# Pyrokine/LineSegmentDetector-SLAM

Hardware: AMD Instinct MI355X
Metric: Mpixels/sec LSD (grad+grow+NFA) (higher is better)
Workload: dtype f64; 1 GPU; 512 x 2048x2048 u8 occupancy maps per GPU tiled/rolled/flipped from 4 aisle-class fixtures (SURVEY 8d C4), full pipeline incl. lineIm, params 0.3/0.6/22.5/0.7/1024; images_total=512, images_rank0=512, parallelism=single GPU, rccl_gather_in_step=False, steps_in_flight=8, steps_in_flight_asked=8, region_waves_per_image=4, help_across_workgroups=False, last_steps_with_help=0, writeback_map=False

## Files before the change

### linesegmentdetector-slam_amd/csrc/k_front.hip

```cpp
#include "lsd_internal.h"
#include "k_front_lds.h"
#include "k1_stage.h"
#include "grad_px.h"

namespace lsdhip {

constexpr int TW = kK1TileW, TH = kK1TileH, NT = 256;
constexpr int GW = kFrontGW, GH = kFrontGH;
constexpr int HS = 17, TAPR = 8;
constexpr int PPT = TW * TH / NT;
static_assert(TW == 32 && TW * TH % NT == 0, "a thread keeps its column and walks down the tile NT / TW rows at a time");

__global__ __launch_bounds__(NT, 4) void k_front(const uint8_t* __restrict__ in, double* __restrict__ mag, double* __restrict__ deg,
                                                 double2* __restrict__ sc, uint32_t* __restrict__ pw, unsigned long long* __restrict__ maxbits,
                                                 int32_t* __restrict__ ties, const double* __restrict__ taps_g, const int* __restrict__ centre_of,
                                                 int W, int H, int w, int h, double gradThre, int IWp, unsigned strip_bytes, unsigned gx,
                                                 unsigned gy, unsigned tiles, uint8_t* __restrict__ clr) {
    extern __shared__ __align__(16) unsigned char smem[];
    double* aux = reinterpret_cast<double*>(smem);
    double* taps = reinterpret_cast<double*>(smem + strip_bytes);
    uint8_t* tile = reinterpret_cast<uint8_t*>(taps + 3 * HS);
    double* Gt = reinterpret_cast<double*>(tile);
    int* l_cnt = reinterpret_cast<int*>(Gt + GW * GH);
    unsigned long long* l_max = reinterpret_cast<unsigned long long*>(l_cnt + 2);
    double2* l_g = reinterpret_cast<double2*>(smem);
    uint32_t* l_px = reinterpret_cast<uint32_t*>(l_g + kFrontList);

    const int tid = threadIdx.x;
    const unsigned per = (tiles + 7u) >> 3;
    const unsigned t = (blockIdx.x & 7u) * per + (blockIdx.x >> 3);
    if (t >= tiles) return;
    const unsigned bx = t % gx, tq = t / gx, by = tq % gy;
    const int X0 = (int)bx * TW, Y0 = (int)by * TH;
    const size_t img = tq / gy;
    const uint8_t* src = in + img * (size_t)W * H;
    const size_t base = img * (size_t)w * h;

    if (clr) {
        typedef uint32_t u32x4 __attribute__((ext_vector_type(4)));
        const unsigned tpi = gx * gy, ti = t % tpi;
        const size_t units = ((size_t)W * H) >> 4;
        const size_t a = units * ti / tpi, e = units * (ti + 1) / tpi;
        u32x4* const v = reinterpret_cast<u32x4*>(clr + img * (size_t)W * H);
        const u32x4 z = {0u, 0u, 0u, 0u};
        for (size_t u = a + tid; u < e; u += NT) __builtin_nontemporal_store(z, &v[u]);
    }
    const int Xf = max(X0 - 1, 0), Yf = max(Y0 - 1, 0);
    const int Xl = min(X0 + TW - 1, w - 1), Yl = min(Y0 + TH - 1, h - 1);
    const int c0 = centre_of[Xf] - TAPR, c1 = centre_of[Xl] + TAPR;
    const int r0 = centre_of[Yf] - TAPR, r1 = centre_of[Yl] + TAPR;
    const int IH = r1 - r0 + 1;

    for (int i = tid; i < 3 * HS; i += NT) taps[i] = taps_g[i];

    const int a0 = c0 - (((c0 % 4) + 4) % 4);
    const uint32_t wany = stage_window(src, tile, W, H, r0, r1, a0, c1, IWp, tid, 0u);

    const int X = tid & (TW - 1), Yt = tid / TW;
    const int gX = X0 + X;
    if (!__syncthreads_or((int)(wany != 0u))) {
        if (gX < w) {
            #pragma unroll
            for (int k = 0; k < PPT; k++) {
                const int gY = Y0 + Yt + k * (NT / TW);
                if (gY >= h) break;
                const GradPx px = grad_pixel(0.0, 0.0, 0.0, 0.0, gX >= 1 && gY >= 1, gradThre);
                const size_t p = base + (size_t)gY * w + gX;
                mag[p] = px.m;
                if (!px.heavy && px.u == 0) sc[p] = make_double2(0.0, 1.0);
                deg[p] = px.d;
                pw[p] = pack_pw(px.d, px.u);
            }
        }
        return;
    }
    const int DWp = IWp >> 2;
    if (gX < w) {
        const int cb = centre_of[gX] - TAPR - a0;
        const double* ker = taps + (gX % 3) * HS;
        double kr[HS];
        #pragma unroll
        for (int i = 0; i < HS; i++) kr[i] = ker[i];
        const uint32_t* trow = reinterpret_cast<const uint32_t*>(tile) + (cb >> 2);
        const uint32_t sh = (uint32_t)(cb & 3);
        for (int r = Yt; r < IH; r += NT / TW) aux[r * GW + 1 + X] = xpass17(trow + r * DWp, sh, kr);
    }
    if (X0 >= 1 && tid < IH) {
        const int cb = centre_of[X0 - 1] - TAPR - a0;
        const double* ker = taps + ((X0 - 1) % 3) * HS;
        double kr[HS];
        #pragma unroll
        for (int i = 0; i < HS; i++) kr[i] = ker[i];
        const uint32_t* trow = reinterpret_cast<const uint32_t*>(tile) + (cb >> 2);
        for (int r = tid; r < IH; r += NT) aux[r * GW] = xpass17(trow + r * DWp, (uint32_t)(cb & 3), kr);
    }
    __syncthreads();
    if (tid == 0) *l_cnt = 0;

    for (int idx = tid; idx < GW * GH; idx += NT) {
        const int Yh = idx / GW, Xh = idx - Yh * GW;
        const int gYh = Y0 - 1 + Yh, gXh = X0 - 1 + Xh;
        const bool ok = gYh >= 0 && gYh < h && gXh >= 0 && gXh < w;
        double v = 0;
        if (ok) {
            const int rb = centre_of[gYh] - TAPR - r0;
            const double* ker = taps + (gYh % 3) * HS;
            double a[HS];
            uint32_t bits = 0u;
            #pragma unroll
            for (int i = 0; i < HS; i++) { a[i] = aux[(rb + i) * GW + Xh]; bits |= (uint32_t)__double2hiint(a[i]) | (uint32_t)__double2loint(a[i]); }
            if (__ballot(bits != 0u) != 0ull) {
                #pragma unroll
                for (int i = 0; i < HS; i++) v += a[i] * ker[i];
            }
        }
        Gt[idx] = v;
    }
    __syncthreads();

    const int lane = tid & 63, wave = tid >> 6;
    const unsigned long long ltmask = (1ull << lane) - 1ull;
    double mx = 0;
    double rowD[PPT];
    uint32_t rowU[PPT];
    int rowSlot[PPT];
    #pragma unroll
    for (int k = 0; k < PPT; k++) {
        const int Y = Yt + k * (NT / TW), gY = Y0 + Y;
        const bool valid = gX < w && gY < h;
        const double* g1 = Gt + (Y + 1) * GW + X;
        const GradPx px = grad_pixel(g1[1], g1[0], g1[1 - GW], g1[-GW], valid && gX >= 1 && gY >= 1, gradThre);
        if (valid) {
            const size_t p = base + (size_t)gY * w + gX;
            mag[p] = px.m;
            if (!px.heavy && px.u == 0) sc[p] = make_double2(0.0, 1.0);
        }
        rowD[k] = px.d; rowU[k] = px.u; rowSlot[k] = -1;
        const unsigned long long hm = __ballot(px.heavy);
        if (hm != 0ull) {
            int b0 = 0;
            if (lane == 0) b0 = atomicAdd(l_cnt, __builtin_popcountll(hm));
            b0 = __builtin_amdgcn_readfirstlane(b0);
            if (px.heavy) {
                const int slot = b0 + __builtin_popcountll(hm & ltmask);
                l_px[slot] = ((uint32_t)(Y * TW + X) << 1) | (px.u == 0 ? 1u : 0u);
                l_g[slot] = make_double2(px.gradX, px.gradY);
                rowSlot[k] = slot;
            }
        }
        mx = fmax(mx, px.m);
    }
    {
        unsigned long long bits = (unsigned long long)__double_as_longlong(mx);
        for (int off = 32; off >= 1; off >>= 1) {
            const unsigned long long o = __shfl_xor(bits, off);
            bits = o > bits ? o : bits;
        }
        if (lane == 0) l_max[wave] = bits;
    }
    __syncthreads();
    if (tid == 0) {
        unsigned long long bits = l_max[0];
        #pragma unroll
        for (int i = 1; i < NT / 64; i++) bits = l_max[i] > bits ? l_max[i] : bits;
        if (bits != 0ull) atomicMax(&maxbits[img], bits);
    }

    const int cnt = *l_cnt;
    for (int i = tid; i < cnt; i += NT) {
        const uint32_t e = l_px[i];
        const double2 gr = l_g[i];
        const double d = grad_angle(gr.x, gr.y, &ties[img]);
        l_g[i] = make_double2(d, 0.0);
        if (e & 1u) {
            const int lt = (int)(e >> 1);
            sc[base + (size_t)(Y0 + lt / TW) * w + (X0 + lt % TW)] = grad_sincos(d);
        }
    }
    __syncthreads();

    if (gX < w) {
        #pragma unroll
        for (int k = 0; k < PPT; k++) {
            const int gY = Y0 + Yt + k * (NT / TW);
            if (gY < h) {
                const double d = rowSlot[k] >= 0 ? l_g[rowSlot[k]].x : rowD[k];
                const size_t p = base + (size_t)gY * w + gX;
                deg[p] = d;
                pw[p] = pack_pw(d, rowU[k]);
            }
        }
    }
}

bool front_fits(const Geom& g, size_t max_lds) {
    if (2 * g.tapR + 1 != HS) return false;
    const size_t need = k_front_lds(g.sca, g.tapR).bytes;
    return need <= 64 * 1024 && need <= max_lds;
}

void launch_front(const Geom& g, const Buffers& b, int n, uint8_t* clr, hipStream_t s) {
    const KFrontLds L = k_front_lds(g.sca, g.tapR);
    const unsigned gx = (g.w + TW - 1) / TW, gy = (g.h + TH - 1) / TH, tiles = gx * gy * (unsigned)n;
    hipLaunchKernelGGL(k_front, dim3(((tiles + 7u) >> 3) * 8u), dim3(NT), L.bytes, s, b.in, b.mag, b.deg, b.sc, b.pw, b.maxbits, b.ties, b.taps,
                       b.centres, g.W, g.H, g.w, g.h, g.gradThre, L.IWp, (unsigned)L.strip, gx, gy, tiles, clr);
}

}
```

### linesegmentdetector-slam_amd/csrc/k_front_lds.h

```cpp
#pragma once
#include <math.h>
#include <stddef.h>
#include "k1_lds.h"

namespace lsdhip {

constexpr int kFrontGW = kK1TileW + 1, kFrontGH = kK1TileH + 1;
constexpr int kFrontList = kK1TileW * kK1TileH;

struct KFrontLds {
    int IWp;
    int IHmax;
    size_t strip;
    size_t window;
    size_t bytes;
};

inline KFrontLds k_front_lds(double sca, int tapR) {
    KFrontLds r;
    const int span = (int)floor(kK1TileW / sca) + 2;
    const int IWmax = span + 2 * tapR + 1;
    r.IWp = ((IWmax + 3) & ~3) + 8;
    if (((r.IWp >> 2) & 1) == 0) r.IWp += 4;
    r.IHmax = (int)floor(kK1TileH / sca) + 2 + 2 * tapR + 1;
    const int hSize = 2 * tapR + 1;
    const size_t sums = (size_t)r.IHmax * kFrontGW * sizeof(double), list = (size_t)kFrontList * (16 + 4);
    const size_t win = ((size_t)r.IHmax * r.IWp + 7) & ~(size_t)7, post = (size_t)kFrontGW * kFrontGH * sizeof(double) + 8 + 4 * 8;
    r.strip = ((sums > list ? sums : list) + 15) & ~(size_t)15;
    r.window = win > post ? win : post;
    r.bytes = r.strip + 3 * (size_t)hSize * sizeof(double) + r.window;
    return r;
}

}
```

### linesegmentdetector-slam_amd/csrc/lsd_ctx.hip

```cpp
#include <math.h>
#include <stddef.h>
#include <stdio.h>
#include <stdlib.h>
#include <string.h>

#include <algorithm>
#include <mutex>
#include <string>
#include <vector>

#include "lsd_devbuf.h"
#include "lsd_internal.h"
#include "k1_lds.h"
#include "k_rdp_lds.h"

using namespace lsdhip;

struct Workspace {
    size_t cap_gpx = 0;
    size_t cap_n = 0, cap_npx = 0, cap_ws = 0;
    int cap_max_lines = 0;
    DevBuf<double> gauss, mag, deg, recs, recs_scaled;
    DevBuf<double2> sc;
    DevBuf<uint32_t> order;
    DevBuf<uint32_t> sets;
    DevBuf<uint32_t> pw, epochmap, ord, spill, gcopy, stamps, seedidx, seedpos, tepoch;
    uint32_t run_id = 0;
    DevBuf<uint32_t> slist;
    DevBuf<double> pend;
    DevBuf<float4> wmeta;
    DevBuf<int> rnum;
    DevBuf<uint32_t> xq;
    DevBuf<unsigned long long> maxbits;
    DevBuf<int32_t> nb, nseed;
    DevBuf<long long> stats;
    DevBuf<SeedRec> seeds;
    int32_t* ties() const { return reinterpret_cast<int32_t*>(maxbits.get() + cap_n); }
};

struct lsd_ctx {
    int device = 0;
    int num_cus = 256;
    size_t max_lds = 0;
    uint32_t id_budget = 0xFFFF0u;
    int tun_soft = 0, tun_claim = 0, tun_feed = 3, tun_big = 0;
    int tun_help = -1;
    int tun_gate = 12000;
    int tun_share = 0;
    int pool_max_images = 4;
    int tun_early = 0, tun_wb = 10, tun_up = 32, tun_down = 96, tun_requeue = 1, tun_xpoll = 20000, tun_linger = 1000000, tun_stop = 0;
    int region_waves_mode = 0;
    bool prefer4 = false;
    hipStream_t stream = nullptr;
    hipStream_t last_stream = nullptr;
    std::string err;
    Workspace ws;
    int mcap = 16384;
    int gcap = 8192;
    DevBuf<uint8_t> h_in, h_lineim;
    DevBuf<lsd_line> h_lines, h_flat;
    DevBuf<int32_t> h_counts, h_offs;
    uint8_t* pin[2] = {nullptr, nullptr};
    hipEvent_t pin_ev[2] = {nullptr, nullptr};
    bool pin_used[2] = {false, false};
    hipStream_t copy_stream = nullptr;
    size_t hcap_n = 0, hcap_wh = 0;
    int hcap_max_lines = 0;
    bool hcap_lineim = false;
    DevBuf<double> d_taps, d_lgamma, d_ptab;
    DevBuf<int> d_centres;
    bool cost_history = false;
    int hist_n = 0;
    lsd_params tab_params{};
    bool tab_valid = false;
    int tapR = 0;
    DevBuf<unsigned long long> mc_claim;
    DevBuf<uint32_t> mc_fa, mc_fb;
    DevBuf<int> mc_ctl;
    DevBuf<uint8_t> mc_in;
    DevBuf<double> mc_out;
    DevBuf<uint8_t> oc_in, oc_out;
    DevBuf<uint8_t> stage;
    DevBuf<uint8_t> fa_buf;
    DevBuf<uint8_t> gm_mr_ws;
    DevBuf<uint32_t> gr_volume;
    DevBuf<uint8_t> gm_slots;
    std::vector<int> fa_nf;
    std::vector<lsd_map_ref> map_tab_host = std::vector<lsd_map_ref>(2 * LSD_MAX_MAPS);
    DevBuf<lsd_map_ref> map_tab;
    int fa_lds_bound = kFaLdsMax;
    DevBuf<int32_t> ga_cnt;
    DevBuf<lsd_line> ga_slab;
    hipEvent_t ga_ev = nullptr;
    bool ga_ev_valid = false;
    int stop_after = 0;
    int tun_groups = -1;
    DevBuf<int> pcount;
    bool trace = false;
    bool fused_front = true;
    int scan_cap = kRdpShortMaxLen;
    bool rdp_long_ready = false;
    int host_max_lines = 8192;
    Geom geom{};
    int last_n = 0;
    int last_max_lines = 0;
    int32_t* last_counts = nullptr;
    bool last_fused = false, last_remapped = false;
    const uint8_t* last_in = nullptr;
    DevBuf<double> dbg_gauss;
    hipEvent_t ev[7]{};
    bool ev_valid = false;
    hipEvent_t ev_done = nullptr;
    bool done_valid = false;
    hipStream_t done_stream = nullptr;
};

constexpr size_t kPinBytes = 32u << 20;

#define HIPCHK(ctx, call)                                                                         \
    do {                                                                                          \
        hipError_t e_ = (call);                                                                   \
        if (e_ != hipSuccess) {                                                                   \
            (ctx)->err = std::string(#call) + ": " + hipGetErrorString(e_);                       \
            return e_ == hipErrorOutOfMemory ? LSD_ERR_NOMEM : LSD_ERR_HIP;                       \
        }                                                                                         \
    } while (0)

static int tap_radius(double sca, double sig) {
    const int prec = 3;
    if (sca < 1) sig = sig / sca;
    return cvt_x86(ceil(sig * sqrt(2 * prec * log(10))));
}

static void gauss_taps(double sca, double sig, int h, std::vector<double>& t) {
    if (sca < 1) sig = sig / sca;
    const int hSize = 1 + 2 * h;
    t.assign((size_t)3 * hSize, 0.0);
    double s1 = 0, s2 = 0, s3 = 0;
    for (int k = 0; k < hSize; k++) {
        const double a = (k - h) / sig, b = (k - h - 1.0 / 3) / sig, c = (k - h + 1.0 / 3) / sig;
        t[0 * hSize + k] = exp(-0.5 * (a * a));
        t[1 * hSize + k] = exp(-0.5 * (b * b));
        t[2 * hSize + k] = exp(-0.5 * (c * c));
        s1 += t[0 * hSize + k]; s2 += t[1 * hSize + k]; s3 += t[2 * hSize + k];
    }
    for (int k = 0; k < hSize; k++) {
        t[0 * hSize + k] /= s1; t[1 * hSize + k] /= s2; t[2 * hSize + k] /= s3;
    }
}

static double log_gamma_host(int x) {
    if (x > 15)
        return 0.918938533204673 + (x - 0.5) * log(x) - x + 0.5 * x * log(x * sinh(1.0 / x) + 1.0 / (810 * pow(x, 6)));
    static const double q[7] = {75122.6331530, 80916.6278952, 36308.2951477, 8687.24529705,
                                1168.92649479, 83.8676043424, 2.50662827511};
    double a = (x + 0.5) * log(x + 5.5) - (x + 5.5), b = 0;
    for (int i = 0; i < 7; i++) { a -= log(x + i); b += q[i] * pow(x, i); }
    return a + log(b);
}

static std::mutex g_lg_mu;
static const double* log_gamma_table(int count) {
    static std::vector<double> tab;
    if ((int)tab.size() < count) {
        const int from = (int)tab.size();
        tab.resize(count);
        for (int i = from; i < count; i++) tab[i] = i >= 1 ? log_gamma_host(i) : 0.0;
    }
    return tab.data();
}

static int make_geom(lsd_ctx* c, const lsd_params* p, int cols, int rows, Geom* g) {
    if (!p || cols <= 0 || rows <= 0) return LSD_ERR_INVALID;
    if (!(p->sca > 0) || !(p->sig > 0) || !(p->angThre > 0) || p->pseBin < 1) return LSD_ERR_INVALID;
    if (p->pseBin > 1024) return LSD_ERR_UNSUPPORTED;
    if (cols > 65535 || rows > 65535) return LSD_ERR_UNSUPPORTED;
    g->W = cols; g->H = rows;
    g->w = cvt_x86(floor(cols * p->sca));
    g->h = cvt_x86(floor(rows * p->sca));
    if (g->w < 2 || g->h < 2) return LSD_ERR_INVALID;
    if (g->w > 32766 || g->h > 32766) return LSD_ERR_UNSUPPORTED;
    if ((long long)g->w * g->h > (1ll << 30)) return LSD_ERR_UNSUPPORTED;
// ... 3 lines not shown
    g->tapR = tap_radius(p->sca, p->sig);
    if (g->tapR < 0 || g->tapR > kMaxTapRadius) return LSD_ERR_UNSUPPORTED;
    const size_t k1_bytes = k1_lds(p->sca, g->tapR).bytes;
    if (k1_bytes > c->max_lds) {
        char msg[200];
        snprintf(msg, sizeof msg, "sca = %g, sig = %g: the Gaussian's window needs %zu bytes of LDS per workgroup, the device has %zu",
                 p->sca, p->sig, k1_bytes, c->max_lds);
        c->err = msg;
        return LSD_ERR_UNSUPPORTED;
    }
    g->pseBin = p->pseBin;
    g->degThre = p->angThre / 180.0 * kPi;
    g->gradThre = 2.0 / sin(g->degThre);
    g->logNT = 5 * (log10(g->h) + log10(g->w)) / 2.0;
    g->regThre = -g->logNT / log10(p->angThre / 180.0);
    g->aliPro = p->angThre / 180.0;
    g->denThre = p->denThre;
    return LSD_OK;
}

static int ensure_tables(lsd_ctx* c, const lsd_params* p, const Geom& g, hipStream_t s) {
    const int lg_need = (int)std::min<long long>(std::max<long long>((long long)g.npx + 2, kLgTable), kLgTableMax);
    if ((int)c->d_lgamma.capacity() < lg_need) {
        HIPCHK(c, hipStreamSynchronize(s));
        if (c->done_valid) HIPCHK(c, hipEventSynchronize(c->ev_done));
        std::lock_guard<std::mutex> lk(g_lg_mu);
        const double* tab = log_gamma_table(lg_need);
        HIPCHK(c, c->d_lgamma.resize(lg_need));
        const hipError_t e = hipMemcpy(c->d_lgamma.get(), tab, sizeof(double) * lg_need, hipMemcpyHostToDevice);
        if (e != hipSuccess) (void)c->d_lgamma.resize(0);
        HIPCHK(c, e);
    }
    if (c->tab_valid && memcmp(&c->tab_params, p, sizeof(lsd_params)) == 0) return LSD_OK;
    if (!c->d_ptab.get()) {
        HIPCHK(c, c->d_ptab.resize(kPTable * 3));
        HIPCHK(c, c->d_taps.resize(3 * (2 * kMaxTapRadius + 1)));
        HIPCHK(c, c->d_centres.resize(kCentreCount));
    }
    std::vector<double> taps;
    gauss_taps(p->sca, p->sig, g.tapR, taps);
    std::vector<int> centres(kCentreCount);
    for (int x = 0; x < kCentreCount; x++) centres[x] = cvt_x86(floor(x / p->sca + 0.5));
    double pt[kPTable * 3];
    double pr = g.aliPro;
    for (int k = 0; k < kPTable; k++) {
        pt[k * 3 + 0] = log(pr); pt[k * 3 + 1] = log10(pr); pt[k * 3 + 2] = log(1 - pr);
        pr /= 2.0;
    }
    HIPCHK(c, hipStreamSynchronize(s));
    if (c->done_valid) HIPCHK(c, hipEventSynchronize(c->ev_done));
    HIPCHK(c, hipMemcpy(c->d_taps.get(), taps.data(), sizeof(double) * taps.size(), hipMemcpyHostToDevice));
    HIPCHK(c, hipMemcpy(c->d_ptab.get(), pt, sizeof(pt), hipMemcpyHostToDevice));
    HIPCHK(c, hipMemcpy(c->d_centres.get(), centres.data(), sizeof(int) * kCentreCount, hipMemcpyHostToDevice));
    c->tab_params = *p;
    c->tab_valid = true;
    c->tapR = g.tapR;
    return LSD_OK;
}

static int waves_for(const lsd_ctx* c, int n) {
    if (c->region_waves_mode == 8 || (c->region_waves_mode == 0 && !c->prefer4 && n <= 4 * c->num_cus)) return 8;
    return 4;
}

constexpr int kPoolHelpMax = 64;
static int pool_for(const lsd_ctx* c, int n, int help) {
    if (help < 0) help = 24;
    if (help > kPoolHelpMax) help = kPoolHelpMax;
    if (help <= 0 || c->trace || n > c->pool_max_images) return 0;
    const int nw = waves_for(c, n);
    const long long free_slots = (long long)(nw == 8 ? 1 : 3) * c->num_cus - n;
    const long long want = ((long long)n * help + nw - 1) / nw;
    const long long p = free_slots < want ? free_slots : want;
    return p > 0 ? (int)p : 0;
}
static int pool_for(const lsd_ctx* c, int n) { return pool_for(c, n, c->tun_help); }
static int pool_reserve_for(const lsd_ctx* c, int n) {
    const int now = c->tun_help < 0 ? 24 : c->tun_help;
    return pool_for(c, n, now > 24 ? now : 24);
}

static bool use_front(const lsd_ctx* c, const Geom& g) {
    return c->fused_front && !c->trace && (c->stop_after == 0 || c->stop_after >= LSD_STAGE_GRAD) && front_fits(g, c->max_lds);
}
static size_t gauss_elems(const lsd_ctx* c, const Geom& g) { return use_front(c, g) ? 0 : (size_t)g.gp * g.h; }

static size_t tm_words(size_t npx) { return npx / 16 + 4 * 8200; }

static int ensure_workspace_impl(lsd_ctx* c, size_t n, size_t npx, size_t gpx, int max_lines, bool trace) {
    Workspace& w = c->ws;
    const size_t need_ws = (n + (size_t)pool_reserve_for(c, (int)n)) * (size_t)waves_for(c, (int)n);
    const bool grow_main = n > w.cap_n || npx > w.cap_npx || gpx > w.cap_gpx || need_ws > w.cap_ws;
    if (grow_main) {
        const size_t nn = n > w.cap_n ? n : w.cap_n, pp = npx > w.cap_npx ? npx : w.cap_npx;
        const size_t gg = gpx > w.cap_gpx ? gpx : w.cap_gpx;
        const size_t ws = need_ws > w.cap_ws ? need_ws : w.cap_ws;
        HIPCHK(c, hipDeviceSynchronize());
        const size_t tot = nn * pp;
        HIPCHK(c, w.gauss.resize(nn * gg)); HIPCHK(c, w.mag.resize(tot)); HIPCHK(c, w.deg.resize(tot));
        HIPCHK(c, w.sc.resize(tot));
        HIPCHK(c, w.pw.resize(tot)); HIPCHK(c, w.epochmap.resize(tot)); HIPCHK(c, w.ord.resize(tot));
        HIPCHK(c, w.spill.resize(ws * pp)); HIPCHK(c, w.gcopy.resize(ws * pp)); HIPCHK(c, w.wmeta.resize(ws * (size_t)c->mcap));
        HIPCHK(c, w.stamps.resize(ws * tm_words(pp))); HIPCHK(c, w.seedidx.resize(tot)); HIPCHK(c, w.seedpos.resize(tot)); HIPCHK(c, w.tepoch.resize(nn * (pp / 16 + 4096)));
        HIPCHK(c, hipMemset(w.stamps.get(), 0, ws * tm_words(pp) * sizeof(uint32_t)));
        HIPCHK(c, hipMemset(w.epochmap.get(), 0, tot * sizeof(uint32_t)));
        w.run_id = 0;
        const size_t gs = ws * (size_t)region_slots();
        HIPCHK(c, w.slist.resize(gs * (size_t)c->gcap));
        HIPCHK(c, w.pend.resize(gs * 24));
        HIPCHK(c, w.order.resize(nn));
        HIPCHK(c, w.sets.resize(nn * 256));
        HIPCHK(c, w.xq.resize(nn * (size_t)(kXStride + 1) + kXHdr));
        HIPCHK(c, w.maxbits.resize(nn + (nn + 1) / 2)); HIPCHK(c, w.nb.resize(nn)); HIPCHK(c, w.nseed.resize(nn));
        HIPCHK(c, w.stats.resize(nn * kStatWords)); HIPCHK(c, w.rnum.resize(nn * (size_t)region_ring() * 2));
        HIPCHK(c, w.seeds.resize(0));
        if (nn != w.cap_n) { w.cap_max_lines = 0; }
        w.cap_n = nn; w.cap_npx = pp; w.cap_gpx = gg; w.cap_ws = ws;
    }
    if (max_lines > w.cap_max_lines) {
        HIPCHK(c, hipDeviceSynchronize());
        HIPCHK(c, w.recs.resize(w.cap_n * (size_t)max_lines * 12));
        HIPCHK(c, w.recs_scaled.resize(w.cap_n * (size_t)max_lines * 4));
        w.cap_max_lines = max_lines;
    }
    if (trace && !w.seeds.get()) {
        HIPCHK(c, hipDeviceSynchronize());
        HIPCHK(c, w.seeds.resize(w.cap_n * w.cap_npx));
    }
    return LSD_OK;
}

static int ensure_workspace(lsd_ctx* c, size_t n, size_t npx, size_t gpx, int max_lines, bool trace) {
    int st = ensure_workspace_impl(c, n, npx, gpx, max_lines, trace);
    if (st != LSD_OK) {
        (void)hipGetLastError();
        c->ws = Workspace{};
        if (st == LSD_ERR_NOMEM && c->region_waves_mode == 0 && !c->prefer4 && waves_for(c, (int)n) == 8) {
            c->prefer4 = true;
            return ensure_workspace(c, n, npx, gpx, max_lines, trace);
        }
    }
    return st;
}

struct Tuning { const char* name; int lo, hi; int lsd_ctx::*field; bool shipped; };
static const Tuning kTunings[] = {
    {"HELP", -1, 4096, &lsd_ctx::tun_help, true},
    {"POOL", 0, 16, &lsd_ctx::pool_max_images, true},
    {"SOFT", 0, 1 << 20, &lsd_ctx::tun_soft, false},
    {"CLAIM", 0, 1 << 20, &lsd_ctx::tun_claim, false},
    {"FEED", 1, 8, &lsd_ctx::tun_feed, false},
    {"BIG", 0, 16, &lsd_ctx::tun_big, false},
    {"EARLY", 0, 4096, &lsd_ctx::tun_early, false},
    {"WB", 0, 100, &lsd_ctx::tun_wb, false},
    {"GATE", 0, 1 << 22, &lsd_ctx::tun_gate, false},
    {"SHARE", 0, 100, &lsd_ctx::tun_share, false},
    {"UP", 0, 1 << 16, &lsd_ctx::tun_up, false},
    {"DOWN", 0, 1 << 16, &lsd_ctx::tun_down, false},
    {"REQUEUE", 0, 1, &lsd_ctx::tun_requeue, false},
    {"XPOLL", 100, 1 << 30, &lsd_ctx::tun_xpoll, false},
    {"LINGER", 1, 1 << 30, &lsd_ctx::tun_linger, false},
    {"GROUPS", -1, 1 << 20, &lsd_ctx::tun_groups, false},
    {"STOP", 0, 1 << 30, &lsd_ctx::tun_stop, false},
    {"FA_LDS", 0, kFaLdsMax, &lsd_ctx::fa_lds_bound, false},
};

// ... 87 lines not shown
    if (c->stream) (void)hipStreamDestroy(c->stream);
    delete c;
}

const char* lsd_last_error(const lsd_ctx* c) { return c ? c->err.c_str() : ""; }
void lsd_free(void* p) { free(p); }

int lsd_set_stop_after(lsd_ctx* c, int stage) {
    if (!c || stage < 0 || stage > LSD_STAGE_REGION) return LSD_ERR_INVALID;
    c->stop_after = stage;
    return LSD_OK;
}
int lsd_set_region_waves(lsd_ctx* c, int waves) {
    if (!c || (waves != 0 && waves != 4 && waves != 8)) return LSD_ERR_INVALID;
    c->region_waves_mode = waves;
    return LSD_OK;
}

int lsd_set_region_help(lsd_ctx* c, int waves) {
    if (!c || waves < -1 || waves > 4096) return LSD_ERR_INVALID;
    c->tun_help = waves;
    return LSD_OK;
}

int lsd_set_cost_history(lsd_ctx* c, int on) {
    if (!c) return LSD_ERR_INVALID;
    c->cost_history = on != 0;
    return LSD_OK;
}

int lsd_debug_set_tuning(lsd_ctx* c, const char* name, int value) {
    if (!c || !name) return LSD_ERR_INVALID;
    for (const Tuning& t : kTunings)
        if (strcmp(name, t.name) == 0) {
            c->*(t.field) = value < t.lo ? t.lo : value > t.hi ? t.hi : value;
            return LSD_OK;
        }
    return LSD_ERR_INVALID;
}

int lsd_debug_set_stamp_budget(lsd_ctx* c, unsigned grows) {
    if (!c || grows < 2u || grows > 0xFFFF0u) return LSD_ERR_INVALID;
    c->id_budget = grows;
    return LSD_OK;
}

int lsd_set_trace(lsd_ctx* c, int on) {
    if (!c) return LSD_ERR_INVALID;
    c->trace = on != 0;
    return LSD_OK;
}

int lsd_set_fused_front(lsd_ctx* c, int on) {
    if (!c) return LSD_ERR_INVALID;
    c->fused_front = on != 0;
    return LSD_OK;
}

int lsd_set_scan_capacity(lsd_ctx* c, int readings) {
    if (!c || readings < kRdpShortMaxLen) return LSD_ERR_INVALID;
    if (readings > LSD_SCAN_MAX_LEN) return LSD_ERR_UNSUPPORTED;
    if (readings > kRdpShortMaxLen && rdp_long_lds(readings) > c->max_lds) {
        char buf[200];
        snprintf(buf, sizeof buf, "scan capacity %d: FeatureScan's work arrays need %zu bytes of LDS, the device gives a workgroup %zu", readings,
                 rdp_long_lds(readings), c->max_lds);
        c->err = buf;
        return LSD_ERR_UNSUPPORTED;
    }
    if (readings != c->scan_cap) { c->scan_cap = readings; c->rdp_long_ready = false; }
    return LSD_OK;
}

int lsd_scan_capacity(const lsd_ctx* c) { return c ? c->scan_cap : LSD_ERR_INVALID; }

int lsd_reserve(lsd_ctx* c, int n, int cols, int rows) {
    if (!c || n <= 0) return LSD_ERR_INVALID;
    lsd_params p; lsd_default_params(&p);
    Geom g;
    int st = make_geom(c, &p, cols, rows, &g);
    if (st != LSD_OK) return st;
    HIPCHK(c, hipSetDevice(c->device));
    st = ensure_workspace(c, (size_t)n, (size_t)g.npx, gauss_elems(c, g), c->ws.cap_max_lines, c->trace);
    if (st != LSD_OK) return st;
    return ensure_tables(c, &p, g, nullptr);
}

int lsd_enqueue_batch_device(lsd_ctx* c, uint8_t* d_maps, int n, int cols, int rows, const lsd_params* p,
                             unsigned flags, uint8_t* d_line_ims, lsd_line* d_lines, int max_lines, int32_t* d_counts,
                             void* stream) {
    if (!c || !d_maps || n <= 0 || !d_lines || !d_counts || max_lines <= 0) return LSD_ERR_INVALID;
    Geom g;
    int st = make_geom(c, p, cols, rows, &g);
    if (st != LSD_OK) return st;
    HIPCHK(c, hipSetDevice(c->device));
    hipStream_t s = (hipStream_t)stream;
    st = ensure_workspace(c, (size_t)n, (size_t)g.npx, gauss_elems(c, g), max_lines, c->trace);
    if (st != LSD_OK) return st;
    st = ensure_tables(c, p, g, s);
    if (st != LSD_OK) return st;
    const bool fused = use_front(c, g);
    if (!fused) HIPCHK(c, prepare_gauss(g));
    if (c->done_valid && c->last_stream != s) HIPCHK(c, hipStreamWaitEvent(s, c->ev_done, 0));

    Workspace& w = c->ws;
    Buffers b{};
    b.in = d_maps;
    b.in_rw = (flags & LSD_FLAG_WRITEBACK_MAP) ? d_maps : nullptr;
    b.gauss = w.gauss.get(); b.mag = w.mag.get(); b.deg = w.deg.get(); b.sc = w.sc.get(); b.pw = w.pw.get(); b.epochmap = w.epochmap.get(); b.sets = w.sets.get(); b.maxbits = w.maxbits.get(); b.nb = w.nb.get(); b.ties = w.ties();
    b.ord = w.ord.get(); b.spill = w.spill.get(); b.gcopy = w.gcopy.get(); b.wmeta = w.wmeta.get(); b.mcap = c->mcap; b.stamps = w.stamps.get(); b.seedidx = w.seedidx.get(); b.seedpos = w.seedpos.get(); b.tepoch = w.tepoch.get();
    b.tm_stride = 4 * ((g.w + 7) >> 3) * ((g.h + 7) >> 3);
    b.order = w.order.get(); b.slist = w.slist.get(); b.gcap = c->gcap; b.id_budget = c->id_budget; b.pend = w.pend.get(); b.rnum = w.rnum.get();
    b.recs = w.recs.get(); b.recs_scaled = w.recs_scaled.get(); b.counts = d_counts; b.lines = d_lines; b.line_im = d_line_ims;
    b.max_lines = max_lines;
    {
        const int nw = waves_for(c, n);
        b.tun_soft = c->tun_soft > 0 ? c->tun_soft : 48 * nw;
        b.tun_claim = c->tun_claim > 0 ? c->tun_claim : 192 * nw;
        b.tun_feed = c->tun_feed;
        b.tun_big = c->tun_big > 0 ? c->tun_big : 3;
        b.tun_help = c->tun_help >= 0 ? c->tun_help : 0;
        b.tun_early = c->tun_early; b.tun_wb = c->tun_wb; b.tun_gate = c->tun_gate; b.tun_share = c->tun_share; b.tun_up = c->tun_up; b.tun_down = c->tun_down; b.tun_requeue = c->tun_requeue;
        b.tun_xpoll = c->tun_xpoll; b.tun_linger = c->tun_linger; b.tun_stop = c->tun_stop;
        b.xq = (b.tun_help > 0 && !c->trace) ? w.xq.get() : nullptr;
        b.npool = b.xq ? pool_for(c, n) : 0;
    }
    b.taps = c->d_taps.get(); b.centres = c->d_centres.get(); b.lgamma = c->d_lgamma.get(); b.lg_count = (int)c->d_lgamma.capacity(); b.ptab = c->d_ptab.get();
    b.seeds = c->trace ? w.seeds.get() : nullptr; b.nseed = w.nseed.get(); b.stats = w.stats.get();

    HIPCHK(c, hipMemsetAsync(w.maxbits.get(), 0, sizeof(unsigned long long) * w.cap_n + sizeof(int32_t) * (size_t)n, s));
    const bool full_region = c->stop_after == 0 || c->stop_after >= LSD_STAGE_REGION;
    if (!full_region) HIPCHK(c, hipMemsetAsync(d_counts, 0, sizeof(int32_t) * n, s));
    if (c->stop_after != 0 && c->stop_after < LSD_STAGE_SORT) HIPCHK(c, hipMemsetAsync(w.nb.get(), 0, sizeof(int32_t) * (size_t)n, s));

    HIPCHK(c, hipEventRecord(c->ev[0], s));
    const bool fused_clear = d_line_ims && (((size_t)cols * rows) & 15) == 0 && (reinterpret_cast<uintptr_t>(d_line_ims) & 15) == 0;
    if (d_line_ims && !fused_clear) launch_clear(d_line_ims, (size_t)n * cols * rows, c->num_cus, s);
    if (fused) launch_front(g, b, n, fused_clear ? d_line_ims : nullptr, s);
    else launch_gauss(g, b, n, fused_clear ? d_line_ims : nullptr, false, s);
    if (b.in_rw) launch_remap_writeback(g, b, n, s);
    HIPCHK(c, hipEventRecord(c->ev[1], s));
    if (!fused && (c->stop_after == 0 || c->stop_after >= LSD_STAGE_GRAD)) launch_gradient(g, b, n, s);
    HIPCHK(c, hipEventRecord(c->ev[2], s));
    if (c->stop_after == 0 || c->stop_after >= LSD_STAGE_SORT) { launch_sort(g, b, n, s); launch_order(b, n, g.npx, (c->cost_history && c->hist_n == n && !c->trace) ? w.stats.get() : nullptr, s); }
    HIPCHK(c, hipEventRecord(c->ev[3], s));
    hipStream_t sr = s;
    if (c->stop_after == 0 || c->stop_after >= LSD_STAGE_REGION) {
        if (++w.run_id >= 1023u) {
            HIPCHK(c, hipMemsetAsync(w.stamps.get(), 0, w.cap_ws * tm_words(w.cap_npx) * sizeof(uint32_t), sr));
            HIPCHK(c, hipMemsetAsync(w.epochmap.get(), 0, w.cap_n * w.cap_npx * sizeof(uint32_t), sr));
            w.run_id = 1;
        }
        if (b.xq) HIPCHK(c, hipMemsetAsync(b.xq, 0, sizeof(uint32_t) * ((size_t)n * (kXStride + 1) + kXHdr), sr));
        const bool wide = waves_for(c, n) == 8;
        int grid = n;
        const int groups = c->tun_groups >= 0 ? c->tun_groups : c->num_cus;
        if (wide && groups > 0 && groups < n && !b.xq && !c->trace) {
            if (!c->pcount.get()) HIPCHK(c, c->pcount.resize(16));
            HIPCHK(c, hipMemsetAsync(c->pcount.get(), 0, sizeof(int), sr));
            b.pcount = c->pcount.get(); b.nimg = n; b.npool = 0;
            grid = groups;
        }
        if (wide) launch_region_w8(g, b, grid, w.run_id << 20, sr);
        else launch_region_w4(g, b, grid, w.run_id << 20, sr);
    }
    HIPCHK(c, hipEventRecord(c->ev[4], s));
    if (c->stop_after == 0) launch_lines(g, b, n, s);
    HIPCHK(c, hipEventRecord(c->ev[5], s));
    HIPCHK(c, hipEventRecord(c->ev_done, s));
    c->done_valid = true; c->done_stream = s;
    HIPCHK(c, hipGetLastError());
    c->ev_valid = true;
    c->hist_n = (c->stop_after == 0 || c->stop_after >= LSD_STAGE_REGION) ? n : 0;
    c->geom = g; c->last_n = n; c->last_max_lines = max_lines; c->last_counts = d_counts; c->last_stream = s;
    c->last_fused = fused; c->last_in = d_maps; c->last_remapped = b.in_rw != nullptr;
    return LSD_OK;
}

int lsd_synchronize(lsd_ctx* c) {
    if (!c) return LSD_ERR_INVALID;
    HIPCHK(c, hipSetDevice(c->device));
    HIPCHK(c, hipStreamSynchronize(c->last_stream));
    return LSD_OK;
}

int lsd_last_timings(lsd_ctx* c, float ms[6]) {
    if (!c || !ms || !c->ev_valid) return LSD_ERR_INVALID;
    HIPCHK(c, hipSetDevice(c->device));
    HIPCHK(c, hipEventSynchronize(c->ev[5]));
    for (int i = 0; i < 5; i++) HIPCHK(c, hipEventElapsedTime(&ms[i], c->ev[i], c->ev[i + 1]));
    HIPCHK(c, hipEventElapsedTime(&ms[5], c->ev[0], c->ev[5]));
    if (c->last_fused) ms[1] = 0.0f;
    return LSD_OK;
}

static int h2d_staged(lsd_ctx* c, void* dst, const void* src, size_t bytes, hipStream_t s) {
    size_t off = 0;
    for (int k = 0; off < bytes; k++) {
        const int b = k & 1;
        const size_t len = bytes - off < kPinBytes ? bytes - off : kPinBytes;
        if (c->pin_used[b]) HIPCHK(c, hipEventSynchronize(c->pin_ev[b]));
        memcpy(c->pin[b], (const uint8_t*)src + off, len);
        HIPCHK(c, hipMemcpyAsync((uint8_t*)dst + off, c->pin[b], len, hipMemcpyHostToDevice, s));
        HIPCHK(c, hipEventRecord(c->pin_ev[b], s));
        c->pin_used[b] = true;
        off += len;
    }
    return LSD_OK;
}
static int d2h_staged(lsd_ctx* c, void* dst, const void* src, size_t bytes, hipStream_t s) {
    size_t off = 0, prev_off = 0, prev_len = 0;
    for (int k = 0; off < bytes; k++) {
        const int b = k & 1;
        const size_t len = bytes - off < kPinBytes ? bytes - off : kPinBytes;
        if (c->pin_used[b] && k < 2) HIPCHK(c, hipEventSynchronize(c->pin_ev[b]));
        HIPCHK(c, hipMemcpyAsync(c->pin[b], (const uint8_t*)src + off, len, hipMemcpyDeviceToHost, s));
        HIPCHK(c, hipEventRecord(c->pin_ev[b], s));
        c->pin_used[b] = true;
        if (prev_len) {
            HIPCHK(c, hipEventSynchronize(c->pin_ev[b ^ 1]));
            memcpy((uint8_t*)dst + prev_off, c->pin[b ^ 1], prev_len);
// ... 1137 lines not shown
```

### linesegmentdetector-slam_amd/csrc/lsd_internal.h

```cpp
#pragma once
#include <hip/hip_runtime.h>
#include <stdint.h>
#include "../../include/lsd_hip.h"

namespace lsdhip {

constexpr double kPi = 3.14159265358979323846;
constexpr int kCentreCount = 32768;
constexpr int kMaxTapRadius = 40;
constexpr int kLgTable = 16384;
constexpr int kLgTableMax = 1 << 23;
constexpr int kStatWords = 48;
constexpr int kStatTiesWord = 39;
constexpr int kStatTotalWord = 8;
constexpr int kPTable = 16;
constexpr int kXStride = 768, kXReq = 64, kXHdr = 16;

struct Geom {
    int W, H;
    int w, h;
    int npx;
    int gp;
    double sca;
    int tapR;
    int pseBin;
    double degThre;
    double gradThre;
    double logNT;
    double regThre;
    double aliPro;
    double denThre;
};

constexpr uint32_t kPwFree = 0u, kPwStatic = 1u, kPwRejected = 2u, kPwLine = 3u;
__host__ __device__ inline uint32_t pw_used(uint32_t w) { return (w & 3u) == 3u ? 1u : (w & 3u); }

struct Buffers {
    const uint8_t* in;
    uint8_t* in_rw;
    double* gauss;
    double* mag;
    double* deg;
    double2* sc;
    uint32_t* pw;
    uint32_t* epochmap;
    uint32_t* sets;
    uint32_t* tepoch;
    unsigned long long* maxbits;
    int32_t* nb;
    int32_t* ties;
    uint32_t* ord;
    uint32_t* stamps;
    int tm_stride;
    uint32_t* spill;
    uint32_t* gcopy;
    float4* wmeta;
    int mcap;
    int* rnum;
    uint32_t* order;
    uint32_t* seedidx;
    uint32_t* seedpos;
    uint32_t* slist;
    int gcap;
    uint32_t id_budget;
    int tun_soft, tun_claim, tun_feed, tun_big;
    uint32_t* xq;
    int tun_help;
    int* pcount;
    int nimg;
    int npool;
    int tun_early;
    int tun_wb;
    int tun_gate;
    int tun_share;
    int tun_up, tun_down;
    int tun_requeue;
    int tun_xpoll;
    int tun_linger;
    int tun_stop;
    double* pend;
    double* recs;
    double* recs_scaled;
    int32_t* counts;
    lsd_line* lines;
    uint8_t* line_im;
    int max_lines;
    const double* taps;
    const int* centres;
    const double* lgamma;
    int lg_count;
    const double* ptab;
    void* seeds;
    int32_t* nseed;
    long long* stats;
};

struct SeedRec {
    int order_idx, x, y, num, outcome, final_num;
    double logNFA;
};

hipError_t prepare_gauss(const Geom& g);
void launch_gauss(const Geom& g, const Buffers& b, int n, uint8_t* clr, bool remapped, hipStream_t s);
bool front_fits(const Geom& g, size_t max_lds);
void launch_front(const Geom& g, const Buffers& b, int n, uint8_t* clr, hipStream_t s);
void launch_remap_writeback(const Geom& g, const Buffers& b, int n, hipStream_t s);
void launch_gradient(const Geom& g, const Buffers& b, int n, hipStream_t s);
void launch_sort(const Geom& g, const Buffers& b, int n, hipStream_t s);
void launch_ordv(const double* mag, const unsigned long long* maxbits, const uint32_t* ord, uint16_t* out, int count, int pseBin, hipStream_t s);
void launch_order(const Buffers& b, int n, int npx, const long long* hist, hipStream_t s);
void launch_region_w4(const Geom& g, const Buffers& b, int n, uint32_t id_base, hipStream_t s);
void launch_region_w8(const Geom& g, const Buffers& b, int n, uint32_t id_base, hipStream_t s);
int region_slots();
int region_waves();
int region_ring();
void launch_calib(double* buf, size_t n, hipStream_t s);
void launch_match(const double* map_cache, int cols, int rows, const lsd_line* map_lines, const lsd_line* scan_lines,
                  const double* pts, int n_points, double lidx, double lidy, double lastx, double lasty, const int* pairs,
                  int n_pairs, double zmax, double max_esti_dist, double* out, hipStream_t s);
void launch_occ_to_map(const uint8_t* in, uint8_t* out, size_t n, hipStream_t s);
void launch_mapcache_spread(const uint8_t* maps, double* out, unsigned long long* claim, uint32_t* fr_a, uint32_t* fr_b, int* ctl,
                            int* cnt, int n, int G, int W, int H, double res, double zmax, int cell_radius, hipStream_t s);
void launch_mapcache(const uint8_t* maps, double* out, unsigned long long* claim, uint32_t* fr_a, uint32_t* fr_b, int n,
                     int W, int H, double res, double zmax, int cell_radius, hipStream_t s);
void launch_lines(const Geom& g, const Buffers& b, int n, hipStream_t s);
void launch_lines_of(const double* recs_scaled, const int32_t* count, lsd_line* lines, uint8_t* line_im, int n, int W, int H, hipStream_t s);
void launch_clear(uint8_t* p, size_t bytes, int num_cus, hipStream_t s);
void launch_compact_lines(const lsd_line* lines, const int32_t* counts, int max_lines, int n, lsd_line* flat, int32_t* offsets, hipStream_t s);
void launch_rdp(const double* scans, const int* lens, int n, int stride, int oriMapCol, int oriMapRow, double mapResol, double mapOriX,
                double mapOriY, int region_point_limit, double thre_line, double line_dist_thre_m, lsd_line* lines_out, int* n_lines,
                double* pts_out, int pts_cap, int* n_pts, double* lidar_pos, int* im_size, hipStream_t s);
void launch_rdp_maps(const double* scans, const int* lens, int n, int stride, const lsd_map_ref* maps, int n_maps, const int32_t* map_of,
                     int scans_per_seq, int region_point_limit, double thre_line, double line_dist_thre_m, lsd_line* lines_out, int* n_lines,
                     double* pts_out, int pts_cap, int* n_pts, double* lidar_pos, int* im_size, hipStream_t s);
int rdp_max_len();
void launch_rdp_long(const double* scans, const int* lens, int n, int stride, double mapResol, double mapOriX, double mapOriY,
                     int region_point_limit, double thre_line, double line_dist_thre_m, lsd_line* lines_out, int* n_lines, double* pts_out,
                     int pts_cap, int* n_pts, double* lidar_pos, int* im_size, hipStream_t s);
void launch_rdp_maps_long(const double* scans, const int* lens, int n, int stride, const lsd_map_ref* maps, int n_maps, const int32_t* map_of,
                          int scans_per_seq, int region_point_limit, double thre_line, double line_dist_thre_m, lsd_line* lines_out,
                          int* n_lines, double* pts_out, int pts_cap, int* n_pts, double* lidar_pos, int* im_size, hipStream_t s);
hipError_t prepare_rdp_long(size_t bytes);
void launch_ingest(const lsd_polar* raw, const float* ranges, const float* min_inc, int n, int n_beams, const int* take, lsd_polar* scans,
                   int* lens, int stride, hipStream_t s);
void launch_grid_integrate(const lsd_polar* scans, const int* lens, int n_scans, int stride, const void* poses, size_t pose_pitch, int cols,
                           int rows, double resol, double range_max, uint32_t* pass, uint32_t* hit, hipStream_t s);
void launch_grid_publish(const uint32_t* pass, const uint32_t* hit, size_t n_cells, uint32_t min_pass, uint32_t occ_num, uint32_t occ_den,
                         int8_t* grid, hipStream_t s);
void launch_grid_likelihood(const uint32_t* pass, const uint32_t* hit, int cols, int rows, uint32_t min_pass, uint32_t occ_num, uint32_t occ_den,
                            const lsd_grid_smear& smear, uint8_t* corr, hipStream_t s);
size_t grid_match_slot_bytes(int n_scans, int na);
void launch_grid_match(const lsd_polar* scans, const int* lens, int n_scans, int stride, const void* poses, size_t pose_pitch, int cols, int rows,
                       double resol, double range_max, const uint8_t* corr, const lsd_grid_search& se, void* slots, lsd_grid_match_rec* out,
                       hipStream_t s);
void launch_grid_match_pick(int n_scans, const void* poses, size_t pose_pitch, const lsd_grid_search& se, const void* slots, lsd_grid_match_rec* out,
                            hipStream_t s);
void launch_grid_coarse(const uint8_t* corr, int cols, int rows, int block, uint8_t* coarse, hipStream_t s);
void grid_match_mr_ws(int n_scans, const lsd_grid_search& se, int block, size_t bytes[4]);
void launch_grid_match_mr(const lsd_polar* scans, const int* lens, int n_scans, int stride, const void* poses, size_t pose_pitch, int cols, int rows,
                          double resol, double range_max, const uint8_t* corr, const uint8_t* coarse, int block, const lsd_grid_search& se,
                          void* const ws[4], lsd_grid_match_rec* out, lsd_grid_match_mr_stats* stats, hipStream_t s);
size_t grid_response_volume_bytes(int n_scans, const lsd_grid_response_par& rp);
void launch_grid_response(const lsd_polar* scans, const int* lens, int n_scans, int stride, const void* poses, size_t pose_pitch,
                          const lsd_grid_match_rec* records, int cols, int rows, double resol, double range_max, const uint8_t* corr, double ang_step,
                          const lsd_grid_response_par& rp, uint32_t* volume, lsd_grid_response_rec* out, hipStream_t s);
void launch_pack_lines(const lsd_line* lines, const int32_t* counts, int n_local, int max_lines, int per, int cap_rows, int32_t* cpad,
                       int32_t* offs, lsd_line* slab, hipStream_t s);
constexpr int kFaCtl = 8, kFaAux = 4, kFaLdsMax = 1024;
struct FaArgs {
    const double* map_cache; int cols, rows;
    const lsd_line* map_lines; int n_map; const int32_t* d_n_map;
    const lsd_line* scan_lines; const int* n_lines; int n_scan_given; int line_pitch;
    const double* pts; const int* n_pts; int n_pts_given; int pts_pitch;
    const double* lidar_pos;
    const int* n_frames; int frames_pitch, t;
    const lsd_position* odom;
    lsd_fa_carry* carry;
    const double* given;
    double map_resol;
    const lsd_map_ref* maps; const int32_t* map_of; int n_maps;
    const lsd_fa_state* init; const lsd_fa_state* state_in;
    lsd_fa_state* states; lsd_fa_report* reports;
    int* pairs; int* n_pairs; int* n_cand; int pair_cap;
    double* cand; int* scratch; double* ctl; double* aux;
    int lds_bound;
};
void launch_fa_frame(const FaArgs& a, int n_seq, bool prepare, hipStream_t s);
void launch_fa_rebase(lsd_fa_carry* carry, int n_seq, const int32_t* key_of, int32_t key, double sc, double tx, double ty, hipStream_t s);
// ... 9 lines not shown
```

Measured before the change: 68240 Mpix/s.

## Precompute tile division plan and exploit periodic tap pattern in front y-pass

```diff
diff --git a/linesegmentdetector-slam_amd/csrc/k_front.hip b/linesegmentdetector-slam_amd/csrc/k_front.hip
--- a/linesegmentdetector-slam_amd/csrc/k_front.hip
+++ b/linesegmentdetector-slam_amd/csrc/k_front.hip
@@ -11,39 +11,77 @@
 constexpr int PPT = TW * TH / NT;
 static_assert(TW == 32 && TW * TH % NT == 0, "a thread keeps its column and walks down the tile NT / TW rows at a time");
 
+__device__ __forceinline__ unsigned div_by(unsigned t, const FrontDiv& d) { return (unsigned)(((unsigned long long)t * d.mul) >> d.shift); }
+
+__device__ __forceinline__ void ypass_block(const double* __restrict__ aux, double* __restrict__ Gt, const double* __restrict__ taps_g, int Xh,
+                                            int b, int rb0, bool colok, int nrow, bool hrow) {
+    double a[27];
+    #pragma unroll
+    for (int j = 0; j < 27; j++) a[j] = 0.0;
+    const double* col = aux + (rb0 - 3) * GW + Xh;
+    if (hrow) {
+        #pragma unroll
+        for (int j = 0; j < 3; j++) a[j] = col[j * GW];
+    }
+    if (colok && nrow > 0) {
+        #pragma unroll
+        for (int j = 3; j < 27; j++) a[j] = col[j * GW];
+    }
+    uint32_t bits = 0u;
+    #pragma unroll
+    for (int j = 0; j < 27; j++) bits |= (uint32_t)__double2hiint(a[j]) | (uint32_t)__double2loint(a[j]);
+    double vh = 0, v0 = 0, v1 = 0, v2 = 0;
+    if (__ballot(bits != 0u) != 0ull) {
+        if (__ballot(hrow) != 0ull) {
+            #pragma unroll
+            for (int i = 0; i < HS; i++) vh += a[i] * taps_g[2 * HS + i];
+        }
+        #pragma unroll
+        for (int i = 0; i < HS; i++) v0 += a[3 + i] * taps_g[i];
+        #pragma unroll
+        for (int i = 0; i < HS; i++) v1 += a[6 + i] * taps_g[HS + i];
+        #pragma unroll
+        for (int i = 0; i < HS; i++) v2 += a[10 + i] * taps_g[2 * HS + i];
+    }
+    double* o = Gt + (1 + 3 * b) * GW + Xh;
+    o[0] = nrow > 0 ? v0 : 0.0; o[GW] = nrow > 1 ? v1 : 0.0; o[2 * GW] = nrow > 2 ? v2 : 0.0;
+    if (b == 0) o[-GW] = hrow ? vh : 0.0;
+}
+
 __global__ __launch_bounds__(NT, 4) void k_front(const uint8_t* __restrict__ in, double* __restrict__ mag, double* __restrict__ deg,
                                                  double2* __restrict__ sc, uint32_t* __restrict__ pw, unsigned long long* __restrict__ maxbits,
                                                  int32_t* __restrict__ ties, const double* __restrict__ taps_g, const int* __restrict__ centre_of,
-                                                 int W, int H, int w, int h, double gradThre, int IWp, unsigned strip_bytes, unsigned gx,
-                                                 unsigned gy, unsigned tiles, uint8_t* __restrict__ clr) {
+                                                 int W, int H, int w, int h, double gradThre, int IWp, unsigned strip_bytes, unsigned flag_off,
+                                                 const FrontPlan P, uint8_t* __restrict__ clr) {
     extern __shared__ __align__(16) unsigned char smem[];
     double* aux = reinterpret_cast<double*>(smem);
     double* taps = reinterpret_cast<double*>(smem + strip_bytes);
     uint8_t* tile = reinterpret_cast<uint8_t*>(taps + 3 * HS);
+    uint32_t* l_any = reinterpret_cast<uint32_t*>(smem + flag_off);
     double* Gt = reinterpret_cast<double*>(tile);
     int* l_cnt = reinterpret_cast<int*>(Gt + GW * GH);
     unsigned long long* l_max = reinterpret_cast<unsigned long long*>(l_cnt + 2);
     double2* l_g = reinterpret_cast<double2*>(smem);
     uint32_t* l_px = reinterpret_cast<uint32_t*>(l_g + kFrontList);
 
-    const int tid = threadIdx.x;
-    const unsigned per = (tiles + 7u) >> 3;
+    const int tid = threadIdx.x, lane = tid & 63, wave = tid >> 6;
+    const unsigned per = (P.tiles + 7u) >> 3;
     const unsigned t = (blockIdx.x & 7u) * per + (blockIdx.x >> 3);
-    if (t >= tiles) return;
-    const unsigned bx = t % gx, tq = t / gx, by = tq % gy;
+    if (t >= P.tiles) return;
+    const unsigned imgu = div_by(t, P.by_tpi), ti = t - imgu * P.tpi;
+    const unsigned by = div_by(ti, P.by_gx), bx = ti - by * P.gx;
     const int X0 = (int)bx * TW, Y0 = (int)by * TH;
-    const size_t img = tq / gy;
+    const size_t img = imgu;
     const uint8_t* src = in + img * (size_t)W * H;
     const size_t base = img * (size_t)w * h;
 
     if (clr) {
         typedef uint32_t u32x4 __attribute__((ext_vector_type(4)));
-        const unsigned tpi = gx * gy, ti = t % tpi;
-        const size_t units = ((size_t)W * H) >> 4;
-        const size_t a = units * ti / tpi, e = units * (ti + 1) / tpi;
+        const unsigned long long a0u = (unsigned long long)ti * P.chunk;
+        const unsigned long long a = a0u < P.units ? a0u : P.units, e = a + P.chunk < P.units ? a + P.chunk : P.units;
         u32x4* const v = reinterpret_cast<u32x4*>(clr + img * (size_t)W * H);
         const u32x4 z = {0u, 0u, 0u, 0u};
-        for (size_t u = a + tid; u < e; u += NT) __builtin_nontemporal_store(z, &v[u]);
+        for (unsigned long long u = a + tid; u < e; u += NT) __builtin_nontemporal_store(z, &v[u]);
     }
     const int Xf = max(X0 - 1, 0), Yf = max(Y0 - 1, 0);
     const int Xl = min(X0 + TW - 1, w - 1), Yl = min(Y0 + TH - 1, h - 1);
@@ -51,14 +89,20 @@
     const int r0 = centre_of[Yf] - TAPR, r1 = centre_of[Yl] + TAPR;
     const int IH = r1 - r0 + 1;
 
-    for (int i = tid; i < 3 * HS; i += NT) taps[i] = taps_g[i];
+    double tapv = 0;
+    if (lane < 3 * HS) tapv = taps_g[lane];
 
     const int a0 = c0 - (((c0 % 4) + 4) % 4);
     const uint32_t wany = stage_window(src, tile, W, H, r0, r1, a0, c1, IWp, tid, 0u);
 
     const int X = tid & (TW - 1), Yt = tid / TW;
     const int gX = X0 + X;
-    if (!__syncthreads_or((int)(wany != 0u))) {
+    {
+        const bool mine = __ballot(wany != 0u) != 0ull;
+        if (lane == 0) l_any[wave] = mine ? 1u : 0u;
+    }
+    __syncthreads();
+    if ((l_any[0] | l_any[1] | l_any[2] | l_any[3]) == 0u) {
         if (gX < w) {
             #pragma unroll
             for (int k = 0; k < PPT; k++) {
@@ -74,6 +118,10 @@
         }
         return;
     }
+    if (lane < 3 * HS) taps[lane] = tapv;
+    __builtin_amdgcn_fence(__ATOMIC_RELEASE, "wavefront");
+    __builtin_amdgcn_wave_barrier();
+    __builtin_amdgcn_fence(__ATOMIC_ACQUIRE, "wavefront");
     const int DWp = IWp >> 2;
     if (gX < w) {
         const int cb = centre_of[gX] - TAPR - a0;
@@ -97,6 +145,17 @@
     __syncthreads();
     if (tid == 0) *l_cnt = 0;
 
+    if (P.ypat) {
+        for (int pass = 0; pass < (wave == NT / 64 - 1 ? 2 : 1); pass++) {
+            const int Xh = pass == 0 ? 1 + X : 0, b = pass == 0 ? Yt : (lane & 7);
+            if (pass == 1 && lane >= 8) break;
+            const int gXh = X0 - 1 + Xh, gY0 = Y0 + 3 * b;
+            const int nrow = min(3, Yl - gY0 + 1);
+            const bool colok = gXh >= 0 && gXh < w;
+            const int rb0 = centre_of[min(gY0, Yl)] - TAPR - r0;
+            ypass_block(aux, Gt, taps_g, Xh, b, rb0, colok, nrow, colok && b == 0 && Y0 >= 1);
+        }
+    } else
     for (int idx = tid; idx < GW * GH; idx += NT) {
         const int Yh = idx / GW, Xh = idx - Yh * GW;
         const int gYh = Y0 - 1 + Yh, gXh = X0 - 1 + Xh;
@@ -118,7 +177,6 @@
     }
     __syncthreads();
 
-    const int lane = tid & 63, wave = tid >> 6;
     const unsigned long long ltmask = (1ull << lane) - 1ull;
     double mx = 0;
     double rowD[PPT];
@@ -129,7 +187,13 @@
         const int Y = Yt + k * (NT / TW), gY = Y0 + Y;
         const bool valid = gX < w && gY < h;
         const double* g1 = Gt + (Y + 1) * GW + X;
-        const GradPx px = grad_pixel(g1[1], g1[0], g1[1 - GW], g1[-GW], valid && gX >= 1 && gY >= 1, gradThre);
+        const double gA = g1[1], gB = g1[0], gC = g1[1 - GW], gD = g1[-GW];
+        const bool interior = valid && gX >= 1 && gY >= 1;
+        const bool some = ((__double2hiint(gA) | __double2loint(gA) | __double2hiint(gB) | __double2loint(gB) | __double2hiint(gC) |
+                            __double2loint(gC) | __double2hiint(gD) | __double2loint(gD)) != 0);
+        GradPx px;
+        if (__ballot(some) == 0ull) px = grad_pixel(0.0, 0.0, 0.0, 0.0, interior, gradThre);
+        else px = grad_pixel(gA, gB, gC, gD, interior, gradThre);
         if (valid) {
             const size_t p = base + (size_t)gY * w + gX;
             mag[p] = px.m;
@@ -199,11 +263,44 @@
     return need <= 64 * 1024 && need <= max_lds;
 }
 
-void launch_front(const Geom& g, const Buffers& b, int n, uint8_t* clr, hipStream_t s) {
+static FrontDiv div_for(unsigned d) {
+    int l = 0;
+    while ((1ull << l) < d) l++;
+    const unsigned long long p = 1ull << (31 + l);
+    return FrontDiv{(unsigned)((p + d - 1) / d), (unsigned)(31 + l)};
+}
+
+bool plan_front(const Geom& g, int n, FrontPlan* out) {
+    FrontPlan P{};
+    const unsigned long long gx = (g.w + TW - 1) / TW, gy = (g.h + TH - 1) / TH, tiles = gx * gy * (unsigned long long)n;
+    if (n <= 0 || gx == 0 || gy == 0 || tiles >= (1ull << 31) - 8) return false;
+    P.gx = (unsigned)gx; P.tpi = (unsigned)(gx * gy); P.tiles = (unsigned)tiles;
+    P.by_tpi = div_for(P.tpi); P.by_gx = div_for(P.gx);
+    P.units = ((unsigned long long)g.W * g.H) >> 4;
+    P.chunk = (P.units + P.tpi - 1) / P.tpi;
+    for (unsigned t = 0; t < P.tiles; t++) {
+        const unsigned img = (unsigned)(((unsigned long long)t * P.by_tpi.mul) >> P.by_tpi.shift), ti = t - img * P.tpi;
+        const unsigned by = (unsigned)(((unsigned long long)ti * P.by_gx.mul) >> P.by_gx.shift), bx = ti - by * P.gx;
+        if (img != t / P.tpi || by != (t % P.tpi) / P.gx || bx != t % P.gx) return false;
+    }
+    if ((unsigned long long)P.tpi * P.chunk < P.units) return false;
+    static_assert(TH % 3 == 0, "a tile's first row has tap phase 0");
+    P.ypat = 1;
+    int prev = cvt_x86(floor(0 / g.sca + 0.5));
+    for (int y = 1; y < g.h && P.ypat; y++) {
+        const int c = cvt_x86(floor(y / g.sca + 0.5));
+        if (c - prev != (y % 3 == 2 ? 4 : 3)) P.ypat = 0;
+        prev = c;
+    }
+    P.n = n; P.w = g.w; P.h = g.h; P.W = g.W; P.H = g.H; P.sca = g.sca;
+    *out = P;
+    return true;
+}
+
+void launch_front(const Geom& g, const Buffers& b, const FrontPlan& P, uint8_t* clr, hipStream_t s) {
     const KFrontLds L = k_front_lds(g.sca, g.tapR);
-    const unsigned gx = (g.w + TW - 1) / TW, gy = (g.h + TH - 1) / TH, tiles = gx * gy * (unsigned)n;
-    hipLaunchKernelGGL(k_front, dim3(((tiles + 7u) >> 3) * 8u), dim3(NT), L.bytes, s, b.in, b.mag, b.deg, b.sc, b.pw, b.maxbits, b.ties, b.taps,
-                       b.centres, g.W, g.H, g.w, g.h, g.gradThre, L.IWp, (unsigned)L.strip, gx, gy, tiles, clr);
-}
-
-}
+    hipLaunchKernelGGL(k_front, dim3(((P.tiles + 7u) >> 3) * 8u), dim3(NT), L.bytes, s, b.in, b.mag, b.deg, b.sc, b.pw, b.maxbits, b.ties, b.taps,
+                       b.centres, g.W, g.H, g.w, g.h, g.gradThre, L.IWp, (unsigned)L.strip, (unsigned)L.flags, P, clr);
+}
+
+}
diff --git a/linesegmentdetector-slam_amd/csrc/k_front_lds.h b/linesegmentdetector-slam_amd/csrc/k_front_lds.h
--- a/linesegmentdetector-slam_amd/csrc/k_front_lds.h
+++ b/linesegmentdetector-slam_amd/csrc/k_front_lds.h
@@ -13,6 +13,7 @@
     int IHmax;
     size_t strip;
     size_t window;
+    size_t flags;
     size_t bytes;
 };
 
@@ -28,7 +29,8 @@
     const size_t win = ((size_t)r.IHmax * r.IWp + 7) & ~(size_t)7, post = (size_t)kFrontGW * kFrontGH * sizeof(double) + 8 + 4 * 8;
     r.strip = ((sums > list ? sums : list) + 15) & ~(size_t)15;
     r.window = win > post ? win : post;
-    r.bytes = r.strip + 3 * (size_t)hSize * sizeof(double) + r.window;
+    r.flags = r.strip + 3 * (size_t)hSize * sizeof(double) + ((r.window + 15) & ~(size_t)15);
+    r.bytes = r.flags + 16;
     return r;
 }
 
diff --git a/linesegmentdetector-slam_amd/csrc/lsd_ctx.hip b/linesegmentdetector-slam_amd/csrc/lsd_ctx.hip
--- a/linesegmentdetector-slam_amd/csrc/lsd_ctx.hip
+++ b/linesegmentdetector-slam_amd/csrc/lsd_ctx.hip
@@ -98,6 +98,7 @@
     DevBuf<int> pcount;
     bool trace = false;
     bool fused_front = true;
+    FrontPlan front_plan{};
     int scan_cap = kRdpShortMaxLen;
     bool rdp_long_ready = false;
     int host_max_lines = 8192;
@@ -267,6 +268,20 @@
 
 static bool use_front(const lsd_ctx* c, const Geom& g) {
     return c->fused_front && !c->trace && (c->stop_after == 0 || c->stop_after >= LSD_STAGE_GRAD) && front_fits(g, c->max_lds);
+}
+static int ensure_front_plan(lsd_ctx* c, const Geom& g, int n) {
+    FrontPlan& P = c->front_plan;
+    if (P.tiles != 0 && n <= P.n && P.w == g.w && P.h == g.h && P.W == g.W && P.H == g.H && P.sca == g.sca) {
+        P.tiles = P.tpi * (unsigned)n;
+        return LSD_OK;
+    }
+    c->front_plan = FrontPlan{};
+    if (!plan_front(g, n, &c->front_plan)) {
+        c->front_plan = FrontPlan{};
+        c->err = "the fused front end's tile arithmetic failed its check against plain division";
+        return LSD_ERR_INTERNAL;
+    }
+    return LSD_OK;
 }
 static size_t gauss_elems(const lsd_ctx* c, const Geom& g) { return use_front(c, g) ? 0 : (size_t)g.gp * g.h; }
 
@@ -520,7 +535,9 @@
     HIPCHK(c, hipSetDevice(c->device));
     st = ensure_workspace(c, (size_t)n, (size_t)g.npx, gauss_elems(c, g), c->ws.cap_max_lines, c->trace);
     if (st != LSD_OK) return st;
-    return ensure_tables(c, &p, g, nullptr);
+    st = ensure_tables(c, &p, g, nullptr);
+    if (st != LSD_OK) return st;
+    return use_front(c, g) ? ensure_front_plan(c, g, n) : LSD_OK;
 }
 
 int lsd_enqueue_batch_device(lsd_ctx* c, uint8_t* d_maps, int n, int cols, int rows, const lsd_params* p,
@@ -538,6 +555,7 @@
     if (st != LSD_OK) return st;
     const bool fused = use_front(c, g);
     if (!fused) HIPCHK(c, prepare_gauss(g));
+    else if ((st = ensure_front_plan(c, g, n)) != LSD_OK) return st;
     if (c->done_valid && c->last_stream != s) HIPCHK(c, hipStreamWaitEvent(s, c->ev_done, 0));
 
     Workspace& w = c->ws;
@@ -573,7 +591,7 @@
     HIPCHK(c, hipEventRecord(c->ev[0], s));
     const bool fused_clear = d_line_ims && (((size_t)cols * rows) & 15) == 0 && (reinterpret_cast<uintptr_t>(d_line_ims) & 15) == 0;
     if (d_line_ims && !fused_clear) launch_clear(d_line_ims, (size_t)n * cols * rows, c->num_cus, s);
-    if (fused) launch_front(g, b, n, fused_clear ? d_line_ims : nullptr, s);
+    if (fused) launch_front(g, b, c->front_plan, fused_clear ? d_line_ims : nullptr, s);
     else launch_gauss(g, b, n, fused_clear ? d_line_ims : nullptr, false, s);
     if (b.in_rw) launch_remap_writeback(g, b, n, s);
     HIPCHK(c, hipEventRecord(c->ev[1], s));
diff --git a/linesegmentdetector-slam_amd/csrc/lsd_internal.h b/linesegmentdetector-slam_amd/csrc/lsd_internal.h
--- a/linesegmentdetector-slam_amd/csrc/lsd_internal.h
+++ b/linesegmentdetector-slam_amd/csrc/lsd_internal.h
@@ -103,7 +103,16 @@
 hipError_t prepare_gauss(const Geom& g);
 void launch_gauss(const Geom& g, const Buffers& b, int n, uint8_t* clr, bool remapped, hipStream_t s);
 bool front_fits(const Geom& g, size_t max_lds);
-void launch_front(const Geom& g, const Buffers& b, int n, uint8_t* clr, hipStream_t s);
+struct FrontDiv { unsigned mul, shift; };
+struct FrontPlan {
+    unsigned gx, tpi, tiles;
+    FrontDiv by_tpi, by_gx;
+    unsigned long long units, chunk;
+    int ypat;
+    int n, w, h, W, H; double sca;
+};
+bool plan_front(const Geom& g, int n, FrontPlan* out);
+void launch_front(const Geom& g, const Buffers& b, const FrontPlan& P, uint8_t* clr, hipStream_t s);
 void launch_remap_writeback(const Geom& g, const Buffers& b, int n, hipStream_t s);
 void launch_gradient(const Geom& g, const Buffers& b, int n, hipStream_t s);
 void launch_sort(const Geom& g, const Buffers& b, int n, hipStream_t s);
```

After: 69210 Mpix/s (median of 6 runs). +1.4%, better.
